# aai-institute/tianshou-fork

Measured on AMD Instinct MI355X. Metric: env-steps/sec through collect+GAE+PPO.learn, higher is better.
Workload: dtype f32 (GAE scan f64)

## Files before the change

include/tsrl.h:

```cpp
#ifndef TSRL_H_
#define TSRL_H_

#include <stdint.h>

#ifdef __cplusplus
extern "C" {
#endif

const char* tsrl_version(void);
const char* tsrl_last_error(void);

int64_t tsrl_gae_workspace_bytes(int64_t n, int64_t row_len);
int64_t tsrl_gae_num_partials(int64_t n, int64_t row_len);
int tsrl_gae(const float* v_s, const float* v_s_next, const double* rew,
             const uint8_t* terminated, const uint8_t* truncated, const uint8_t* end_extra,
             int64_t n, int64_t row_len, const double* value_scale, double gamma,
             double gae_lambda, float* adv_out, float* ret_out, double* adv64_out,
             double* ret64_out, double* ret_partials, void* workspace,
             int64_t workspace_bytes, void* stream);

int tsrl_gae_f64v(const double* v_s, const double* v_s_next, const double* rew,
                  const uint8_t* terminated, const uint8_t* truncated, const uint8_t* end_extra,
                  int64_t n, int64_t row_len, double gamma, double gae_lambda,
                  double* adv64_out, double* ret64_out, void* workspace,
// ... 186 lines not shown
    double eps_clip;
    double dual_clip;
    double vf_coef;
    double ent_coef;
    double adv_eps;
    double b_global;
    int32_t value_clip;
    int32_t norm_adv;
    int32_t objective;
    int32_t pad_;
} tsrl_ppo_params;

int64_t tsrl_ppo_num_partials(int64_t b);
int tsrl_adv_moments(const float* adv, const int64_t* idx, int64_t b, double* partials,
                     void* stream);
int64_t tsrl_adv_moments_seg_parts(int64_t max_seg);
int tsrl_adv_moments_seg(const float* adv, const int64_t* idx, const int64_t* bounds,
                         int64_t nseg, int64_t max_seg, double* partials, double* out,
                         void* stream);
int tsrl_reduce_partials(const double* partials, int64_t nblk, int64_t width, double* out,
                         void* stream);
int tsrl_ppo_gauss_fwd_bwd(const float* mu, const float* log_std, const float* value,
                           const float* act, const float* logp_old, const float* adv,
                           const float* ret, const float* v_s, const int64_t* idx,
                           int64_t b, int64_t act_dim, const double* adv_sums,
                           tsrl_ppo_params p, float* grad_mu, float* grad_value,
                           double* partials, void* stream);
int tsrl_ppo_gauss_finalize(const double* sums, int64_t act_dim, const float* log_std,
                            tsrl_ppo_params p, float* losses, float* grad_log_std,
                            void* stream);
int tsrl_gauss_logp(const float* mu, const float* log_std, const float* act, int64_t b,
                    int64_t act_dim, float* out, void* stream);

int tsrl_ppo_cat_fwd_bwd(const float* x, const float* value, const int64_t* act,
                         const float* logp_old, const float* adv, const float* ret,
                         const float* v_s, const int64_t* idx, int64_t b, int64_t num_actions,
                         int mode, const double* adv_sums, tsrl_ppo_params p, float* grad_x,
                         float* grad_value, double* partials, void* stream);
int tsrl_ppo_cat_finalize(const double* sums, tsrl_ppo_params p, float* losses, void* stream);
int tsrl_cat_logp(const float* x, const int64_t* act, int64_t b, int64_t num_actions, int mode,
                  float* out, void* stream);

int tsrl_cat_gumbel_argmax(const float* logits, const float* u, int64_t n, int64_t num_actions,
                           int64_t* out, void* stream);

typedef struct tsrl_tail_weights {
    const float *w2a, *b2a;
    const float *w2c, *b2c;
    const float *w3a, *b3a;
    const float *w3c, *b3c;
    const float *log_std;
} tsrl_tail_weights;

typedef struct tsrl_tail_grads {
    float *w2a, *b2a, *w2c, *b2c, *w3a, *b3a, *w3c, *b3c;
} tsrl_tail_grads;

int tsrl_mlp_l1_fwd(const float* X, int64_t ldx, const int64_t* idx, int64_t n, int64_t D,
                    const float* Wa, const float* ba, const float* Wc, const float* bc,
                    int act_tanh, float* out, int frag_out, void* stream);
int64_t tsrl_mlp_frag_floats(int64_t n);
int64_t tsrl_mlp_split_bytes(int64_t D);
int tsrl_mlp_split_w(const float* Wa, const float* Wc, int64_t D, void* wsplit, void* stream);
int tsrl_mlp_l1_fwd_x6(const float* X, int64_t ldx, const int64_t* idx, int64_t n, int64_t D,
                       const void* wsplit, const float* ba, const float* bc, int act_tanh,
                       float* out, int frag_out, void* stream);
int64_t tsrl_ppo_tail_workspace_bytes(int64_t n);
int tsrl_ppo_tail_stage(const float* h1frag, int64_t n, const int64_t* idx,
                        const tsrl_tail_weights* w, int64_t act_dim, const float* act,
                        const float* logp_old, const float* adv, const float* ret,
                        const float* v_s, const double* adv_sums, tsrl_ppo_params p, float* dz1,
                        const tsrl_tail_grads* grads, double* sums, void* workspace,
                        int64_t ws_bytes, const float* log_std, float* losses,
                        float* grad_log_std, int stages, void* stream);
int tsrl_ppo_eval(const float* h1frag, int64_t n, const tsrl_tail_weights* w, int64_t act_dim,
                  const float* act, float* value_out, float* logp_out, void* stream);

int64_t tsrl_ppo_eval_fused_workspace_bytes(void);
int tsrl_ppo_eval_fused(const float* X, int64_t ldx, const int64_t* idx, int64_t n, int64_t D,
                        const void* wsplit, const float* ba, const float* bc,
                        const tsrl_tail_weights* wt, int64_t act_dim, const float* act,
                        float* value_out, float* logp_out, void* workspace, int64_t ws_bytes,
                        void* stream);
int64_t tsrl_mlp_dw_workspace_bytes(int64_t n, int64_t D);
int tsrl_mlp_dw(const float* dz1, const float* X, int64_t ldx, const int64_t* idx, int64_t n,
                int64_t D, float* gWa, float* gba, float* gWc, float* gbc, void* workspace,
                int64_t ws_bytes, void* stream);

int64_t tsrl_policy_pack_floats(int64_t D);
int tsrl_policy_pack_l1(const float* W, int64_t D, float* packed, void* stream);
int tsrl_gauss_policy_act(const float* obs, int64_t ldx, int64_t n, int64_t D,
                          const float* w1packed, const float* b1, const float* w2,
                          const float* b2, const float* w3, const float* b3,
                          const float* log_std, int64_t act_dim, const float* eps,
                          int bound_method, const float* low, const float* high, float* act,
                          float* act_remap, void* stream);
int tsrl_gauss_policy_act_rng(const float* obs, int64_t ldx, int64_t n, int64_t D,
                              const float* w1packed, const float* b1, const float* w2,
                              const float* b2, const float* w3, const float* b3,
                              const float* log_std, int64_t act_dim, uint64_t seed,
                              const int64_t* rng_ctr, int64_t* rng_next, int bound_method,
                              const float* low, const float* high, float* act,
                              float* act_remap, void* stream);

int tsrl_nstep_return(const double* rew, const uint8_t* done, const uint8_t* terminated,
                      const int64_t* last_index, const int64_t* lengths, int64_t size,
                      int64_t num, const int64_t* idx, int64_t bsz, int64_t n_step,
                      double gamma, const void* target_q, int64_t X, int f64, void* out,
                      void* stream);
int tsrl_segtree_set(double* tree, int64_t bound, const int64_t* idx, const double* values,
                     int64_t value_stride, int64_t k, int* win, void* stream);
int tsrl_segtree_reduce(const double* tree, int64_t bound, int64_t start, int64_t end,
                        double* out, void* stream);
int tsrl_segtree_prefix_idx(const double* tree, int64_t bound, const void* values, int f64,
                            int64_t k, int64_t* out, void* stream);

typedef struct {
    void* out;
    int64_t off_a, off_c, d, kp;
} tsrl_w1_split;
int64_t tsrl_clip_adam_partials(int64_t n);
int tsrl_clip_adam(float* param, float* grad, float* exp_avg, float* exp_avg_sq, int64_t n,
                   float* step, int64_t nstep, float lr, float beta1, float beta2, float eps,
                   float max_norm, double* partials, float* norm_out, unsigned int* ticket,
                   const float* lr_dev, const tsrl_w1_split* split, int scale_grads,
                   void* stream);
int tsrl_clip_rmsprop(float* param, float* grad, float* square_avg, int64_t n, float* step,
                      int64_t nstep, float lr, float alpha, float eps, float max_norm,
                      double* partials, float* norm_out, unsigned int* ticket,
                      const float* lr_dev, const tsrl_w1_split* split, int scale_grads,
                      void* stream);

int tsrl_dqn_target_q(const float* q_sel, const float* q_eval, int64_t b, int64_t num_actions,
                      int is_double, float* out, void* stream);
int64_t tsrl_dqn_num_partials(int64_t b);
int tsrl_dqn_td_fwd_bwd(const float* q, const int64_t* act, const float* returns,
                        const float* weight, int64_t b, int64_t num_actions, int huber,
                        float* grad_q, float* td_error, double* partials, float* loss,
                        void* stream);
int tsrl_eps_greedy(int64_t* act, const double* u_row, const double* u_act,
                    const uint8_t* mask, double eps, int64_t n, int64_t num_actions,
                    void* stream);

#ifdef __cplusplus
}
#endif
#endif
```

tianshou-fork_amd/csrc/mlp.hip:

```cpp
#include "ppo_loss.h"
#include "x6.h"

namespace tsrl {
namespace {

typedef float f32x16 __attribute__((ext_vector_type(16)));
using x6::bf16x8;
using x6::mfma6;
using x6::NPL;
using x6::split1;
using x6::sw_off;

constexpr int H = 64;
constexpr int HC = 2 * H;
constexpr int NT = HC / 32;
constexpr int AMAX = 32;

__device__ __forceinline__ int rho(int r) { return (r & 3) + 8 * (r >> 2); }

__device__ __forceinline__ f32x16 mfma(float a, float b, f32x16 c) {
    return __builtin_amdgcn_mfma_f32_32x32x2f32(a, b, c, 0, 0, 0);
}

__device__ __forceinline__ f32x16 zero16() {
// ... 749 lines not shown
            __builtin_amdgcn_sched_barrier(0);
            run_net(bt, 0, ua);
            __builtin_amdgcn_sched_barrier(0);
            if (bt + bstep < ntiles) load_unit(bt + bstep, 0, ua);
            __builtin_amdgcn_sched_barrier(0);
            run_net(bt, 1, ub);
            __builtin_amdgcn_sched_barrier(0);
        }
    } else {
        for (; bt < ntiles; bt += bstep) {
            float h1[2][16];
            load_unit(bt, 1, h1);
            run_net(bt, 1, h1);
        }
    }
}

struct TailGrads {
    float *w2a, *b2a, *w2c, *b2c, *w3a, *b3a, *w3c, *b3c;
};

template <typename T>
__device__ __forceinline__ T slab_sum(const T* __restrict__ base, int64_t stride, int nslab,
                                      int64_t i, bool valid, T* sh) {
    const int o = threadIdx.x & 63, g = threadIdx.x >> 6;
    T a0 = 0, a1 = 0, a2 = 0, a3 = 0;
    if (valid) {
        int k = g;
        for (; k + 12 < nslab; k += 16) {
            a0 += base[(int64_t)k * stride + i];
            a1 += base[(int64_t)(k + 4) * stride + i];
            a2 += base[(int64_t)(k + 8) * stride + i];
            a3 += base[(int64_t)(k + 12) * stride + i];
        }
        for (; k < nslab; k += 4) a0 += base[(int64_t)k * stride + i];
    }
    sh[g * 64 + o] = (a0 + a1) + (a2 + a3);
    __syncthreads();
    return ((sh[o] + sh[64 + o]) + sh[128 + o]) + sh[192 + o];
}

struct TailFin {
    const float* log_std;
    float* losses;
    float* grad_log_std;
    float vf_coef, ent_coef;
    double inv_b;
};

__global__ __launch_bounds__(256) void tail_reduce_kernel(const float* __restrict__ slab_f,
                                                          const double* __restrict__ slab_d,
                                                          int nslab, int A, TailGrads g,
                                                          double* __restrict__ sums, TailFin fin) {
    __shared__ float shf[256];
    __shared__ double shd[256];
    const int nfb = (SL_F + 63) / 64;
    if ((int)blockIdx.x < nfb) {
        const int i = blockIdx.x * 64 + (threadIdx.x & 63);
        const float s = slab_sum(slab_f, SL_F, nslab, i, i < SL_F, shf);
        if (threadIdx.x >= 64 || i >= SL_F) return;
        if (i < SL_B2A) g.w2a[i] = s;
        else if (i < SL_W2C) g.b2a[i - SL_B2A] = s;
        else if (i < SL_B2C) g.w2c[i - SL_W2C] = s;
        else if (i < SL_W3A) g.b2c[i - SL_B2C] = s;
        else if (i < SL_B3A) { if (i - SL_W3A < A * H) g.w3a[i - SL_W3A] = s; }
        else if (i < SL_W3C) { if (i - SL_B3A < A) g.b3a[i - SL_B3A] = s; }
        else if (i < SL_B3C) g.w3c[i - SL_W3C] = s;
        else if (i == SL_B3C) g.b3c[0] = s;
    } else {
        const int k0 = threadIdx.x & 63;
        const double s = slab_sum(slab_d, SL_D, nslab, k0, k0 < SL_D, shd);
        if (threadIdx.x < 64 && k0 < 4 + A) sums[k0] = s;
        if (fin.losses) {
            __shared__ double fs[64];
            if (threadIdx.x < 64) fs[k0] = s;
            __syncthreads();
            gauss_finalize(fs, A, fin.log_std, fin.vf_coef, fin.ent_coef, fin.inv_b, fin.losses,
                           fin.grad_log_std);
        }
    }
}

constexpr int DW_COLS = 128;
constexpr int DW_KB = 32;

#ifndef DWX6_OCC
#define DWX6_OCC 2
#endif
__global__ __launch_bounds__(256, DWX6_OCC) void dw_x6_kernel(
    const float* __restrict__ dz, const float* __restrict__ X, int64_t ldx,
    const int64_t* __restrict__ idx, int64_t n, int D, int64_t rows_per_split, int ncolpad,
    int ncolt, float* __restrict__ part) {
    constexpr int PL = 128 * 64;
    __shared__ __attribute__((aligned(16))) char Zi[NPL * PL];
    __shared__ __attribute__((aligned(16))) char Xi[NPL * PL];
    const int t = threadIdx.x;
    const int w = t >> 6, l = t & 63, h = l >> 5, c = l & 31;
    const int G = gridDim.x, b = blockIdx.x;
    const int L = (G & 7) ? b : (b & 7) * (G >> 3) + (b >> 3);
    const int colt = L % ncolt, split = L / ncolt;
    const int col0 = colt * DW_COLS;
    const int64_t r0 = (int64_t)split * rows_per_split;
    const int64_t r1 = min(n, r0 + rows_per_split);
    const int fc = t & 127;
    const int rg = __builtin_amdgcn_readfirstlane(t >> 7);
    const int k = col0 + fc;
    const float ones = k == D ? 1.0f : 0.0f;
    const bool kin = k < D;
    const float* xcol = X + (kin ? k : 0);
    const uint64_t ldx32 = (uint32_t)ldx;
    float zr[16], xr[16];
#define DWX6_LOAD(rb)                                                                       \
    {                                                                                       \
        _Pragma("unroll") for (int q = 0; q < 16; ++q) {                                    \
            const int64_t r = (rb) + 8 * (rg + 2 * (q >> 3)) + (q & 7);                     \
            const int64_t rr = r < r1 ? r : r1 - 1;                                          \
            const int64_t ri = idx ? idx[rr] : rr;                                          \
            zr[q] = dz[rr * HC + fc];                                                       \
            xr[q] = xcol[ri * ldx];                                                         \
        }                                                                                   \
    }
     \
     \
     \
     \
#define DWX6_LOAD_FULL(rb)                                                                  \
    {                                                                                       \
        _Pragma("unroll") for (int g_ = 0; g_ < 2; ++g_) {                                  \
            const int64_t rg0_ = (rb) + 8 * (rg + 2 * g_);                                  \
            const float* zb_ = dz + rg0_ * HC + fc;                                         \
            const int64_t* ib_ = idx + rg0_;                                                \
            _Pragma("unroll") for (int j_ = 0; j_ < 8; ++j_) {                              \
                zr[8 * g_ + j_] = zb_[j_ * HC];                                             \
                const uint64_t ri_ = (uint32_t)ib_[j_];                                     \
                xr[8 * g_ + j_] = xcol[ri_ * ldx32];                                        \
            }                                                                               \
        }                                                                                   \
    }
     \
     \
#define DWX6_STORE(rb, FULL)                                                                \
    {                                                                                       \
        _Pragma("unroll") for (int g = 0; g < 2; ++g) {                                     \
            bf16x8 zp[NPL], xp[NPL];                                                        \
            _Pragma("unroll") for (int j = 0; j < 8; ++j) {                                 \
                const bool lv = (FULL) || (rb) + 8 * (rg + 2 * g) + j < r1;                 \
                const float zv = lv ? zr[8 * g + j] : 0.0f;                                 \
                const float xv = lv ? (kin ? xr[8 * g + j] : ones) : 0.0f;                  \
                __bf16 a0, a1, a2;                                                          \
                split1(zv, a0, a1, a2);                                                     \
                zp[0][j] = a0;                                                              \
                zp[1][j] = a1;                                                              \
                zp[2][j] = a2;                                                              \
                split1(xv, a0, a1, a2);                                                     \
                xp[0][j] = a0;                                                              \
                xp[1][j] = a1;                                                              \
                xp[2][j] = a2;                                                              \
            }                                                                               \
            const int off = sw_off(fc, rg + 2 * g);                                         \
            _Pragma("unroll") for (int p = 0; p < NPL; ++p) {                               \
                *reinterpret_cast<bf16x8*>(Zi + p * PL + off) = zp[p];                      \
                *reinterpret_cast<bf16x8*>(Xi + p * PL + off) = xp[p];                      \
            }                                                                               \
        }                                                                                   \
    }
    f32x16 acc[NT];
#pragma unroll
    for (int i = 0; i < NT; ++i) acc[i] = zero16();
    const int64_t nchunk = r1 > r0 ? (r1 - r0 + DW_KB - 1) / DW_KB : 0;
    if (nchunk > 0) {
        DWX6_LOAD(r0)
        DWX6_STORE(r0, false)
    }
    __syncthreads();
    for (int64_t ch = 0; ch < nchunk; ++ch) {
        if (ch + 1 < nchunk) {
            const int64_t rb = r0 + (ch + 1) * DW_KB;
            if (idx && rb + DW_KB <= r1)
                DWX6_LOAD_FULL(rb)
            else
                DWX6_LOAD(rb)
        }
#pragma unroll
        for (int s = 0; s < 2; ++s) {
            bf16x8 b[NPL];
            const int xo = sw_off(32 * w + c, 2 * s + h);
#pragma unroll
            for (int p = 0; p < NPL; ++p) b[p] = *reinterpret_cast<const bf16x8*>(Xi + p * PL + xo);
#pragma unroll
            for (int i = 0; i < NT; ++i) {
                bf16x8 a[NPL];
                const int zo = sw_off(32 * i + c, 2 * s + h);
#pragma unroll
                for (int p = 0; p < NPL; ++p)
                    a[p] = *reinterpret_cast<const bf16x8*>(Zi + p * PL + zo);
                acc[i] = mfma6(a, b, acc[i]);
            }
        }
        if (ch + 1 < nchunk) {
            __syncthreads();
            const int64_t rb = r0 + (ch + 1) * DW_KB;
            if (rb + DW_KB <= r1)
                DWX6_STORE(rb, true)
            else
                DWX6_STORE(rb, false)
            __syncthreads();
        }
    }
#undef DWX6_LOAD
#undef DWX6_LOAD_FULL
#undef DWX6_STORE
    float* o = part + (int64_t)split * HC * ncolpad;
#pragma unroll
    for (int i = 0; i < NT; ++i)
#pragma unroll
        for (int r = 0; r < 16; ++r)
            o[(int64_t)(32 * i + rho(r) + 4 * h) * ncolpad + col0 + 32 * w + c] = acc[i][r];
}

__global__ __launch_bounds__(256) void dw_reduce_kernel(const float* __restrict__ part,
                                                        int nsplit, int ncolpad, int D,
                                                        float* __restrict__ gWa,
                                                        float* __restrict__ gba,
                                                        float* __restrict__ gWc,
                                                        float* __restrict__ gbc) {
    __shared__ float sh[256];
    const int64_t i = (int64_t)blockIdx.x * 64 + (threadIdx.x & 63);
    const int64_t total = (int64_t)HC * ncolpad;
    const int f = (int)(i / ncolpad), k = (int)(i - (int64_t)f * ncolpad);
    const bool valid = i < total && k <= D;
    const float s = slab_sum(part, total, nsplit, i, valid, sh);
    if (threadIdx.x >= 64 || !valid) return;
    if (k == D) {
        if (f < H) gba[f] = s; else gbc[f - H] = s;
    } else {
        if (f < H) gWa[(int64_t)f * D + k] = s; else gWc[(int64_t)(f - H) * D + k] = s;
    }
}

int tail_grid(int64_t n) {
    const int64_t tiles = (n + 15) / 16;
    const int64_t g = (tiles + T16_NW - 1) / T16_NW;
    return (int)std::min<int64_t>(g, 256);
}

int dw_nsplit(int64_t n) {
    int64_t s = std::max<int64_t>(1, std::min<int64_t>(170, n / 64));
    if (s >= 8) s &= ~int64_t(7);
    return (int)s;
}

}
}

using namespace tsrl;

extern "C" int tsrl_mlp_l1_fwd(const float* X, int64_t ldx, const int64_t* idx, int64_t n,
                               int64_t D, const float* Wa, const float* ba, const float* Wc,
                               const float* bc, int act_tanh, float* out, int frag_out,
                               void* stream) {
    TSRL_CHECK_ARG(n >= 0 && D > 0 && ldx >= D, "tsrl_mlp_l1_fwd: bad sizes");
    if (n == 0) return 0;
    TSRL_CHECK_ARG(X && Wa && ba && Wc && bc && out, "tsrl_mlp_l1_fwd: null pointer");
    TSRL_CHECK_ARG(aligned16(X) && ldx % 4 == 0 && aligned16(Wa) && aligned16(Wc) && D % 4 == 0 &&
                       aligned16(out),
                   "tsrl_mlp_l1_fwd: X/W/out must be 16-byte aligned with D, ldx multiples of 4");
    const unsigned grid = (unsigned)((n + L1_ROWS - 1) / L1_ROWS);
    hipLaunchKernelGGL(l1_fwd_kernel, dim3(grid), dim3(256), 0, as_stream(stream), X, ldx, idx, n,
                       (int)D, Wa, ba, Wc, bc, act_tanh, out, frag_out);
    TSRL_LAUNCH_CHECK("tsrl_mlp_l1_fwd");
    return 0;
}

extern "C" int64_t tsrl_mlp_frag_floats(int64_t n) {
    return ((n + L1_ROWS - 1) / L1_ROWS) * L1_ROWS * HC;
}

extern "C" int64_t tsrl_ppo_tail_workspace_bytes(int64_t n) {
    const int g = tail_grid(n);
    return (int64_t)g * (SL_F * (int64_t)sizeof(float) + SL_D * (int64_t)sizeof(double)) + 256;
}

extern "C" int tsrl_ppo_tail_stage(const float* h1frag, int64_t n, const int64_t* idx,
                                   const tsrl_tail_weights* wt, int64_t act_dim, const float* act,
                                   const float* logp_old, const float* adv, const float* ret,
                                   const float* v_s, const double* adv_sums, tsrl_ppo_params prm,
                                   float* dz1, const tsrl_tail_grads* grads, double* sums,
                                   void* workspace, int64_t ws_bytes, const float* log_std,
                                   float* losses, float* grad_log_std, int stages, void* stream) {
    TSRL_CHECK_ARG((log_std && losses && grad_log_std) || (!log_std && !losses && !grad_log_std),
                   "tsrl_ppo_tail_stage: log_std/losses/grad_log_std all set or all null");
    TSRL_CHECK_ARG((stages >= 1 && stages <= 3) || stages == 4 || stages == 8,
                   "tsrl_ppo_tail_stage: stages must be 1, 2, 3, 4 or 8");
    TSRL_CHECK_ARG(n > 0 && act_dim > 0 && act_dim <= AMAX,
                   "tsrl_ppo_tail_stage: need n > 0 and 0 < act_dim <= %d", AMAX);
    TSRL_CHECK_ARG(h1frag && wt && grads && act && adv && ret && dz1 && sums && workspace,
                   "tsrl_ppo_tail_stage: null pointer");
    TSRL_CHECK_ARG(objective_args_ok(prm, logp_old),
                   "tsrl_ppo_tail_stage: objective 0 needs logp_old; objective 1 takes no "
                   "norm_adv, value_clip or dual_clip");
    TSRL_CHECK_ARG(!prm.value_clip || v_s, "tsrl_ppo_tail_stage: value_clip needs v_s");
    TSRL_CHECK_ARG(!prm.norm_adv || adv_sums, "tsrl_ppo_tail_stage: norm_adv needs adv_sums");
    TSRL_CHECK_ARG(prm.b_global >= 1.0, "tsrl_ppo_tail_stage: b_global < 1");
    TSRL_CHECK_ARG(ws_bytes >= tsrl_ppo_tail_workspace_bytes(n),
                   "tsrl_ppo_tail_stage: workspace too small");
    TSRL_CHECK_ARG(aligned16(h1frag) && aligned16(dz1),
                   "tsrl_ppo_tail_stage: h1frag/dz1 not 16-byte aligned");
    const int g = tail_grid(n);
    float* slab_f = reinterpret_cast<float*>(workspace);
    uintptr_t dptr = reinterpret_cast<uintptr_t>(slab_f + (int64_t)g * SL_F);
    dptr = (dptr + 15) & ~(uintptr_t)15;
    double* slab_d = reinterpret_cast<double*>(dptr);
    TailWeights w{wt->w2a, wt->b2a, wt->w2c, wt->b2c, wt->w3a, wt->b3a, wt->w3c, wt->b3c,
                  wt->log_std};
    const LossParams lp = make_loss_params(prm);
    const int A = (int)act_dim;
    if (stages & (1 | 4)) {
        auto actor = prm.objective == OBJ_A2C ? ppo_tail16_kernel<0, OBJ_A2C>
                                              : ppo_tail16_kernel<0, OBJ_PPO>;
        hipLaunchKernelGGL(actor, dim3(g), dim3(T16_TPB), 0, as_stream(stream), h1frag, n, idx,
                           w, act, logp_old, adv, ret, v_s, adv_sums, lp, A, dz1, slab_f, slab_d);
        TSRL_LAUNCH_CHECK("tsrl_ppo_tail_stage(actor)");
    }
    if (stages & (1 | 8)) {
        hipLaunchKernelGGL((ppo_tail16_kernel<1, OBJ_PPO>), dim3(g), dim3(T16_TPB), 0,
                           as_stream(stream), h1frag, n, idx, w, act, logp_old, adv, ret, v_s,
                           adv_sums, lp, A, dz1, slab_f, slab_d);
        TSRL_LAUNCH_CHECK("tsrl_ppo_tail_stage(critic)");
    }
    if (!(stages & 2)) return 0;
    TailGrads gg{grads->w2a, grads->b2a, grads->w2c, grads->b2c, grads->w3a, grads->b3a,
                 grads->w3c, grads->b3c};
    const TailFin fin{log_std, losses, grad_log_std, lp.vf_coef, lp.ent_coef, lp.inv_b};
    hipLaunchKernelGGL(tail_reduce_kernel, dim3((SL_F + 63) / 64 + 1), dim3(256), 0,
                       as_stream(stream), slab_f, slab_d, g, A, gg, sums, fin);
    TSRL_LAUNCH_CHECK("tsrl_ppo_tail_stage(reduce)");
    return 0;
}

extern "C" int64_t tsrl_mlp_dw_workspace_bytes(int64_t n, int64_t D) {
    const int ncolpad = (int)(((D + 1 + DW_COLS - 1) / DW_COLS) * DW_COLS);
    const int nsplit = dw_nsplit(n);
    return (int64_t)nsplit * HC * ncolpad * (int64_t)sizeof(float);
}

extern "C" int tsrl_mlp_dw(const float* dz1, const float* X, int64_t ldx, const int64_t* idx,
                           int64_t n, int64_t D, float* gWa, float* gba, float* gWc, float* gbc,
                           void* workspace, int64_t ws_bytes, void* stream) {
    TSRL_CHECK_ARG(n > 0 && D > 0 && ldx >= D, "tsrl_mlp_dw: bad sizes");
    TSRL_CHECK_ARG(dz1 && X && gWa && gba && gWc && gbc && workspace, "tsrl_mlp_dw: null pointer");
    TSRL_CHECK_ARG(aligned16(dz1) && aligned16(X) && ldx % 4 == 0 && ldx >= (D + 3) / 4 * 4 && ldx < (int64_t(1) << 32),
                   "tsrl_mlp_dw: dz1/X must be 16-byte aligned, ldx a multiple of 4 and >= "
                   "roundup(D, 4) (columns D.. of the padding read as data-free)");
    TSRL_CHECK_ARG(ws_bytes >= tsrl_mlp_dw_workspace_bytes(n, D), "tsrl_mlp_dw: workspace too small");
    const int ncolt = (int)((D + 1 + DW_COLS - 1) / DW_COLS);
    const int ncolpad = ncolt * DW_COLS;
    const int nsplit = dw_nsplit(n);
    const int64_t rps = ((n + nsplit - 1) / nsplit + DW_KB - 1) / DW_KB * DW_KB;
    float* part = reinterpret_cast<float*>(workspace);
    hipLaunchKernelGGL(dw_x6_kernel, dim3(ncolt * nsplit), dim3(256), 0, as_stream(stream),
                       dz1, X, ldx, idx, n, (int)D, rps, ncolpad, ncolt, part);
    TSRL_LAUNCH_CHECK("tsrl_mlp_dw");
    const int64_t outs = (int64_t)HC * ncolpad;
    hipLaunchKernelGGL(dw_reduce_kernel, dim3((unsigned)((outs + 63) / 64)), dim3(256), 0,
                       as_stream(stream), part, nsplit, ncolpad, (int)D, gWa, gba, gWc, gbc);
    TSRL_LAUNCH_CHECK("tsrl_mlp_dw(reduce)");
    return 0;
}

extern "C" int tsrl_ppo_eval(const float* h1frag, int64_t n, const tsrl_tail_weights* wt,
                             int64_t act_dim, const float* act, float* value_out,
                             float* logp_out, void* stream) {
    TSRL_CHECK_ARG(n >= 0 && act_dim > 0 && act_dim <= AMAX, "tsrl_ppo_eval: bad sizes");
    if (n == 0) return 0;
    TSRL_CHECK_ARG(h1frag && wt && value_out && (!logp_out || act),
                   "tsrl_ppo_eval: null pointer");
    TSRL_CHECK_ARG(aligned16(h1frag), "tsrl_ppo_eval: h1frag not 16-byte aligned");
    TailWeights w{wt->w2a, wt->b2a, wt->w2c, wt->b2c, wt->w3a, wt->b3a, wt->w3c, wt->b3c,
                  wt->log_std};
    const int64_t tiles = (n + 31) / 32;
    const unsigned g = (unsigned)std::min<int64_t>((tiles + 3) / 4, 1024);
    if (logp_out)
        hipLaunchKernelGGL(eval_tail_kernel<true>, dim3(g), dim3(256), 0, as_stream(stream), h1frag,
                           n, w, (int)act_dim, act, value_out, logp_out);
    else
        hipLaunchKernelGGL(eval_tail_kernel<false>, dim3(g), dim3(256), 0, as_stream(stream),
                           h1frag, n, w, (int)act_dim, act, value_out, logp_out);
    TSRL_LAUNCH_CHECK("tsrl_ppo_eval");
    return 0;
}
```

tianshou-fork_amd/tianshou_amd/_C.py:

```python
import ctypes
import os

import torch

_HERE = os.path.dirname(os.path.abspath(__file__))
LIB_PATH = os.environ.get("TSRL_LIB_PATH") or os.path.join(_HERE, "lib", "libtsrl.so")

_i64 = ctypes.c_int64
_u64 = ctypes.c_uint64
_p = ctypes.c_void_p
_d = ctypes.c_double
_f = ctypes.c_float
_i32 = ctypes.c_int32


class AddArgs(ctypes.Structure):
    _fields_ = [
        ("ids", _p), ("ptr", _p), ("next_rel", _p), ("offset", _p), ("k", _i64),
        ("uniform_rel", _i64), ("uniform_next", _i64), ("rel_dev", _p), ("ring_size", _i64),
        ("obs_src", _p), ("obs_dst", _p), ("obs_row_bytes", _i64),
        ("obs_next_src", _p), ("obs_next_dst", _p), ("cur_obs", _p), ("obs_dim", _i64),
        ("norm_mean", _p), ("norm_var", _p), ("norm_eps", _f), ("norm_clip", _f),
        ("obs_next_src_raw", _p), ("obs_next_dst_raw", _p),
        ("act_src", _p), ("act_dst", _p), ("act_row_bytes", _i64),
# ... 85 lines not shown
    "tsrl_rms_sum_partials2": ([_p, _p, _p, _i64, _i64, _i64, _p, _p], ctypes.c_int),
    "tsrl_rms_norm_rows": ([_p, _p, _i64, _i64, _p, _p, _f, _f, _p, _p], ctypes.c_int),
    "tsrl_buffer_add": ([ctypes.POINTER(AddArgs), _p], ctypes.c_int),
    "tsrl_collect_pack_floats": ([_i64], _i64),
    "tsrl_collect_pack_w1": ([_p, _i64, _p, _p], ctypes.c_int),
    "tsrl_collect_workspace_bytes": ([_i64, _i64], _i64),
    "tsrl_collect_box_step": ([ctypes.POINTER(CollectArgs), _p], ctypes.c_int),
    "tsrl_collect_rms_finalize": ([ctypes.POINTER(CollectArgs), _p], ctypes.c_int),
    "tsrl_collect_totals_offset": ([_i64], _i64),
    "tsrl_collect_spec_step": ([ctypes.POINTER(CollectArgs), _i32, _p], ctypes.c_int),
    "tsrl_collect_xpipe_finalize": ([ctypes.POINTER(CollectArgs), _p], ctypes.c_int),
    "tsrl_rms_exact_stats_bytes": ([_i64], _i64),
    "tsrl_rms_exact_stats": ([_p, _i64, _p, _p, _i64, _p, _p], ctypes.c_int),
    "tsrl_rms_exact_stats_n": ([_i32, _p, _p, _p, _i64, _i64, _p, _p], ctypes.c_int),
    "tsrl_rms_exact_stats_max_steps": ([], ctypes.c_int),
    "tsrl_gather_rows": ([_p, _i64, _p, _i64, _p, _p], ctypes.c_int),
    "tsrl_gather_rows_pitched": ([_p, _i64, _i64, _p, _i64, _p, _p], ctypes.c_int),
    "tsrl_np_shuffle_draws": ([_p, _p, _i64, _p], ctypes.c_int),
    "tsrl_shuffle_apply_workspace_bytes": ([_i64], _i64),
    "tsrl_shuffle_apply": ([_p, _i64, _p, _p, _i64, _p], ctypes.c_int),
    "tsrl_ring_step_index": ([_p, _i64, _p, _p, _p, _i64, _i64, ctypes.c_int, _p, _p],
                             ctypes.c_int),
    "tsrl_stack_gather_pitched": ([_p, _i64, _i64, _p, _i64, _i64, _p, _p, _p, _i64, _i64, _p,
                                   _p, _p], ctypes.c_int),
    "tsrl_stack_gather": ([_p, _i64, _p, _i64, _i64, _p, _p, _p, _i64, _i64, _p, _p, _p],
                          ctypes.c_int),
    "tsrl_frames_to_f32_nhwc": ([_p, _i64, _i64, _i64, _p, _p, _p], ctypes.c_int),
    "tsrl_dqn_conv1_fwd": ([_p, _i64, _p, _p, _i64, _i64, _i64, _i64, _p, _f, ctypes.c_int, _p,
                            _p],
                           ctypes.c_int),
    "tsrl_dqn_conv2_dgrad": ([_p, _i64, _p, _i64, _i64, _i64, _i64, _p, _p, _p], ctypes.c_int),
    "tsrl_relu_bwd_rows_workspace_bytes": ([_i64, _i64], _i64),
    "tsrl_relu_bwd_rows": ([_p, _p, _p, _i64, _i64, _p, _p, _i64, _p], ctypes.c_int),
    "tsrl_bias_relu_rows": ([_p, _p, _i64, _i64, _p], ctypes.c_int),
    "tsrl_dqn_conv1_wgrad_workspace_bytes": ([_i64], _i64),
    "tsrl_dqn_conv1_wgrad": ([_p, _i64, _p, _p, _f, _p, _p, _p, _i64, _p], ctypes.c_int),
    "tsrl_nstep_return": ([_p, _p, _p, _p, _p, _i64, _i64, _p, _i64, _i64, _d, _p, _i64,
                           ctypes.c_int, _p, _p], ctypes.c_int),
    "tsrl_clip_adam_partials": ([_i64], _i64),
    "tsrl_clip_adam": ([_p, _p, _p, _p, _i64, _p, _i64, _f, _f, _f, _f, _f, _p, _p, _p, _p,
                        ctypes.POINTER(W1Split), ctypes.c_int, _p],
                       ctypes.c_int),
    "tsrl_clip_rmsprop": ([_p, _p, _p, _i64, _p, _i64, _f, _f, _f, _f, _p, _p, _p, _p,
                           ctypes.POINTER(W1Split), ctypes.c_int, _p], ctypes.c_int),
    "tsrl_segtree_set": ([_p, _i64, _p, _p, _i64, _i64, _p, _p], ctypes.c_int),
    "tsrl_segtree_reduce": ([_p, _i64, _i64, _i64, _p, _p], ctypes.c_int),
    "tsrl_segtree_prefix_idx": ([_p, _i64, _p, ctypes.c_int, _i64, _p, _p], ctypes.c_int),
    "tsrl_sum_rows_workspace_bytes": ([_i64, _i64], _i64),
    "tsrl_sum_rows_f32": ([_p, _i64, _i64, _p, _p, _i64, _p], ctypes.c_int),
    "tsrl_ppo_num_partials": ([_i64], _i64),
    "tsrl_adv_moments": ([_p, _p, _i64, _p, _p], ctypes.c_int),
    "tsrl_reduce_partials": ([_p, _i64, _i64, _p, _p], ctypes.c_int),
    "tsrl_adv_moments_seg_parts": ([_i64], _i64),
    "tsrl_adv_moments_seg": ([_p, _p, _p, _i64, _i64, _p, _p, _p], ctypes.c_int),
    "tsrl_ppo_gauss_fwd_bwd": ([_p, _p, _p, _p, _p, _p, _p, _p, _p, _i64, _i64, _p, PPOParams,
                                _p, _p, _p, _p], ctypes.c_int),
    "tsrl_ppo_gauss_finalize": ([_p, _i64, _p, PPOParams, _p, _p, _p], ctypes.c_int),
    "tsrl_gauss_logp": ([_p, _p, _p, _i64, _i64, _p, _p], ctypes.c_int),
    "tsrl_ppo_cat_fwd_bwd": ([_p, _p, _p, _p, _p, _p, _p, _p, _i64, _i64, ctypes.c_int, _p,
                              PPOParams, _p, _p, _p, _p], ctypes.c_int),
    "tsrl_ppo_cat_finalize": ([_p, PPOParams, _p, _p], ctypes.c_int),
    "tsrl_cat_logp": ([_p, _p, _i64, _i64, ctypes.c_int, _p, _p], ctypes.c_int),
    "tsrl_cat_gumbel_argmax": ([_p, _p, _i64, _i64, _p, _p], ctypes.c_int),
    "tsrl_rms_exact_update": ([_p, _p, _i64, _p, _p, _i64, _i64, _p, _p, _p, _p, _p, _p, _p],
                              ctypes.c_int),
    "tsrl_np_shuffle_draws_mt": ([_p, _p, _i64, _p, ctypes.c_int], ctypes.c_int),
    "tsrl_mlp_l1_fwd": ([_p, _i64, _p, _i64, _i64, _p, _p, _p, _p, ctypes.c_int, _p,
                         ctypes.c_int, _p], ctypes.c_int),
    "tsrl_mlp_frag_floats": ([_i64], _i64),
    "tsrl_mlp_split_bytes": ([_i64], _i64),
    "tsrl_mlp_split_w": ([_p, _p, _i64, _p, _p], ctypes.c_int),
    "tsrl_mlp_l1_fwd_x6": ([_p, _i64, _p, _i64, _i64, _p, _p, _p, ctypes.c_int, _p,
                            ctypes.c_int, _p], ctypes.c_int),
    "tsrl_ppo_tail_workspace_bytes": ([_i64], _i64),
    "tsrl_ppo_tail_stage": ([_p, _i64, _p, ctypes.POINTER(TailWeights), _i64, _p, _p, _p, _p,
                             _p, _p, PPOParams, _p, ctypes.POINTER(TailGrads), _p, _p, _i64, _p,
                             _p, _p, ctypes.c_int, _p], ctypes.c_int),
    "tsrl_ppo_eval": ([_p, _i64, ctypes.POINTER(TailWeights), _i64, _p, _p, _p, _p],
                      ctypes.c_int),
    "tsrl_ppo_eval_fused_workspace_bytes": ([], _i64),
    "tsrl_ppo_eval_fused": ([_p, _i64, _p, _i64, _i64, _p, _p, _p, ctypes.POINTER(TailWeights),
                             _i64, _p, _p, _p, _p, _i64, _p], ctypes.c_int),
    "tsrl_mlp_dw_workspace_bytes": ([_i64, _i64], _i64),
    "tsrl_policy_pack_floats": ([_i64], _i64),
    "tsrl_gauss_policy_act_rng": ([_p, _i64, _i64, _i64, _p, _p, _p, _p, _p, _p, _p, _i64, _u64,
                                   _p, _p, ctypes.c_int, _p, _p, _p, _p, _p], ctypes.c_int),
    "tsrl_policy_pack_l1": ([_p, _i64, _p, _p], ctypes.c_int),
    "tsrl_gauss_policy_act": ([_p, _i64, _i64, _i64, _p, _p, _p, _p, _p, _p, _p, _i64, _p,
                               ctypes.c_int, _p, _p, _p, _p, _p], ctypes.c_int),
    "tsrl_mlp_dw": ([_p, _p, _i64, _p, _i64, _i64, _p, _p, _p, _p, _p, _i64, _p], ctypes.c_int),
    "tsrl_dqn_target_q": ([_p, _p, _i64, _i64, ctypes.c_int, _p, _p], ctypes.c_int),
    "tsrl_dqn_num_partials": ([_i64], _i64),
    "tsrl_dqn_td_fwd_bwd": ([_p, _p, _p, _p, _i64, _i64, ctypes.c_int, _p, _p, _p, _p, _p],
                            ctypes.c_int),
    "tsrl_eps_greedy": ([_p, _p, _p, _p, _d, _i64, _i64, _p], ctypes.c_int),
}

EXPORTED = tuple(_SIGS)
_LIB = None


class TsrlError(RuntimeError):
    pass


def lib():
    global _LIB
    if _LIB is None:
        if not os.path.exists(LIB_PATH):
            raise ImportError(
                f"libtsrl.so not found at {LIB_PATH}: build it with "
                "`python -c 'import __graft_entry__ as g; g.build()'` (hipcc, gfx950)")
        L = ctypes.CDLL(LIB_PATH)
        for name, (args, res) in _SIGS.items():
            fn = getattr(L, name)
            fn.argtypes = args
            fn.restype = res
        _LIB = L
    return _LIB


def check(rc, what=""):
    if rc != 0:
        msg = lib().tsrl_last_error().decode(errors="replace")
        raise TsrlError(f"{what or 'libtsrl'} failed (hipError {rc}): {msg}")


def stream_ptr(device=None):
    return torch.cuda.current_stream(device).cuda_stream


def ptr(t, dtype=None):
    if t is None:
        return None
    if not isinstance(t, torch.Tensor):
        raise TypeError(f"expected a torch.Tensor, got {type(t)}")
    if t.device.type != "cuda":
        raise TsrlError(f"libtsrl kernels need HIP device tensors; got a tensor on {t.device}")
    if dtype is not None and t.dtype != dtype:
        raise TypeError(f"expected dtype {dtype}, got {t.dtype}")
    if not t.is_contiguous():
        raise ValueError("libtsrl kernels need contiguous tensors")
    return t.data_ptr()


def ptr_rows(t):
    if t is None:
        return None
    if t.dim() >= 2 and t[0].is_contiguous() and t.stride(0) >= t[0].numel():
        if t.device.type != "cuda":
            raise TsrlError(f"libtsrl kernels need HIP device tensors; got a tensor on {t.device}")
        return t.data_ptr()
    return ptr(t)
```

Baseline: 68.20 million.

## Widen MLP weight-gradient kernel to multi-column-tile blocks with double-buffered LDS

Replaces the dW kernel with a templated wide kernel in which one block covers up to three 128-column tiles. The dz tile is loaded and split once per block and reused across those column tiles instead of being reloaded per tile. The chunk size drops to 16 rows, with double-buffered LDS images, register prefetch two chunks ahead, and split/MFMA interleaving via sched_group_barrier, so only one barrier is needed per chunk. The cost is larger blocks (up to 768 threads), more LDS and registers per block, a possible second launch for leftover tiles, and a new plan API.

```diff
diff --git a/include/tsrl.h b/include/tsrl.h
--- a/include/tsrl.h
+++ b/include/tsrl.h
@@ -292,6 +292,8 @@
                         const tsrl_tail_weights* wt, int64_t act_dim, const float* act,
                         float* value_out, float* logp_out, void* workspace, int64_t ws_bytes,
                         void* stream);
+int tsrl_mlp_dw_plan(int64_t n, int64_t D, int64_t* nsplit, int64_t* rows_per_split,
+                     int64_t* col_tiles, int64_t* chunk_rows);
 int64_t tsrl_mlp_dw_workspace_bytes(int64_t n, int64_t D);
 int tsrl_mlp_dw(const float* dz1, const float* X, int64_t ldx, const int64_t* idx, int64_t n,
                 int64_t D, float* gWa, float* gba, float* gWc, float* gbc, void* workspace,
diff --git a/tianshou-fork_amd/csrc/mlp.hip b/tianshou-fork_amd/csrc/mlp.hip
--- a/tianshou-fork_amd/csrc/mlp.hip
+++ b/tianshou-fork_amd/csrc/mlp.hip
@@ -855,134 +855,189 @@
 }
 
 constexpr int DW_COLS = 128;
-constexpr int DW_KB = 32;
-
-#ifndef DWX6_OCC
-#define DWX6_OCC 2
-#endif
-__global__ __launch_bounds__(256, DWX6_OCC) void dw_x6_kernel(
+constexpr int DW_KB = 16;
+constexpr int DW_MAXCT = 3;
+
+__device__ __forceinline__ int dw_off(int row, int q) {
+    return row * 32 + 16 * (q ^ ((row >> 2) & 1) ^ ((row >> 3) & 1));
+}
+
+template <int CT>
+__global__ __launch_bounds__(256 * CT) void dw_wide_kernel(
     const float* __restrict__ dz, const float* __restrict__ X, int64_t ldx,
     const int64_t* __restrict__ idx, int64_t n, int D, int64_t rows_per_split, int ncolpad,
-    int ncolt, float* __restrict__ part) {
-    constexpr int PL = 128 * 64;
-    __shared__ __attribute__((aligned(16))) char Zi[NPL * PL];
-    __shared__ __attribute__((aligned(16))) char Xi[NPL * PL];
+    int colt0, int ngrp, float* __restrict__ part) {
+    constexpr int NC = DW_COLS * CT;
+    constexpr int NS = 2;
+    constexpr int ZPL = HC * 2 * DW_KB;
+    constexpr int XPL = NC * 2 * DW_KB;
+    constexpr int BUF = NPL * (ZPL + XPL);
+    __shared__ __attribute__((aligned(16))) char img[2 * BUF];
     const int t = threadIdx.x;
     const int w = t >> 6, l = t & 63, h = l >> 5, c = l & 31;
-    const int G = gridDim.x, b = blockIdx.x;
-    const int L = (G & 7) ? b : (b & 7) * (G >> 3) + (b >> 3);
-    const int colt = L % ncolt, split = L / ncolt;
-    const int col0 = colt * DW_COLS;
+    const int grp = blockIdx.x % ngrp, split = blockIdx.x / ngrp;
+    const int col0 = (colt0 + grp * CT) * DW_COLS;
     const int64_t r0 = (int64_t)split * rows_per_split;
     const int64_t r1 = min(n, r0 + rows_per_split);
-    const int fc = t & 127;
-    const int rg = __builtin_amdgcn_readfirstlane(t >> 7);
-    const int k = col0 + fc;
+    const int xc = t % NC;
+    const int xrg = __builtin_amdgcn_readfirstlane(t / NC);
+    const bool zt = __builtin_amdgcn_readfirstlane(w) < 4;
+    const int zf = t & 127;
+    const int zrg = __builtin_amdgcn_readfirstlane((t >> 7) & 1);
+    const int k = col0 + xc;
     const float ones = k == D ? 1.0f : 0.0f;
     const bool kin = k < D;
-    const float* xcol = X + (kin ? k : 0);
+    const uint32_t kxb = (kin ? k : 0) * 4u, zfb = zf * 4u;
+    auto at = [](const float* row, uint32_t byte_off) __attribute__((always_inline)) {
+        return *reinterpret_cast<const float*>(reinterpret_cast<const char*>(row) + byte_off);
+    };
     const uint64_t ldx32 = (uint32_t)ldx;
-    float zr[16], xr[16];
-#define DWX6_LOAD(rb)                                                                       \
-    {                                                                                       \
-        _Pragma("unroll") for (int q = 0; q < 16; ++q) {                                    \
-            const int64_t r = (rb) + 8 * (rg + 2 * (q >> 3)) + (q & 7);                     \
-            const int64_t rr = r < r1 ? r : r1 - 1;                                          \
-            const int64_t ri = idx ? idx[rr] : rr;                                          \
-            zr[q] = dz[rr * HC + fc];                                                       \
-            xr[q] = xcol[ri * ldx];                                                         \
-        }                                                                                   \
-    }
-     \
-     \
-     \
-     \
-#define DWX6_LOAD_FULL(rb)                                                                  \
-    {                                                                                       \
-        _Pragma("unroll") for (int g_ = 0; g_ < 2; ++g_) {                                  \
-            const int64_t rg0_ = (rb) + 8 * (rg + 2 * g_);                                  \
-            const float* zb_ = dz + rg0_ * HC + fc;                                         \
-            const int64_t* ib_ = idx + rg0_;                                                \
-            _Pragma("unroll") for (int j_ = 0; j_ < 8; ++j_) {                              \
-                zr[8 * g_ + j_] = zb_[j_ * HC];                                             \
-                const uint64_t ri_ = (uint32_t)ib_[j_];                                     \
-                xr[8 * g_ + j_] = xcol[ri_ * ldx32];                                        \
-            }                                                                               \
-        }                                                                                   \
-    }
-     \
-     \
-#define DWX6_STORE(rb, FULL)                                                                \
-    {                                                                                       \
-        _Pragma("unroll") for (int g = 0; g < 2; ++g) {                                     \
-            bf16x8 zp[NPL], xp[NPL];                                                        \
-            _Pragma("unroll") for (int j = 0; j < 8; ++j) {                                 \
-                const bool lv = (FULL) || (rb) + 8 * (rg + 2 * g) + j < r1;                 \
-                const float zv = lv ? zr[8 * g + j] : 0.0f;                                 \
-                const float xv = lv ? (kin ? xr[8 * g + j] : ones) : 0.0f;                  \
-                __bf16 a0, a1, a2;                                                          \
-                split1(zv, a0, a1, a2);                                                     \
-                zp[0][j] = a0;                                                              \
-                zp[1][j] = a1;                                                              \
-                zp[2][j] = a2;                                                              \
-                split1(xv, a0, a1, a2);                                                     \
-                xp[0][j] = a0;                                                              \
-                xp[1][j] = a1;                                                              \
-                xp[2][j] = a2;                                                              \
-            }                                                                               \
-            const int off = sw_off(fc, rg + 2 * g);                                         \
-            _Pragma("unroll") for (int p = 0; p < NPL; ++p) {                               \
-                *reinterpret_cast<bf16x8*>(Zi + p * PL + off) = zp[p];                      \
-                *reinterpret_cast<bf16x8*>(Xi + p * PL + off) = xp[p];                      \
-            }                                                                               \
-        }                                                                                   \
-    }
+    int wsz[2], wsx[2], rdz[2], rdx[2];
+#pragma unroll
+    for (int q = 0; q < 2; ++q) {
+        wsz[q] = q * BUF + dw_off(zf, zrg);
+        wsx[q] = q * BUF + NPL * ZPL + dw_off(xc, xrg);
+        rdz[q] = q * BUF + dw_off(c, h);
+        rdx[q] = q * BUF + NPL * ZPL + dw_off(32 * w + c, h);
+        asm volatile("" : "+v"(wsz[q]), "+v"(wsx[q]), "+v"(rdz[q]), "+v"(rdx[q]));
+    }
+
+    auto load_full = [&](float (&xs)[8], float (&zs)[8], int64_t rb, bool zt) __attribute__((always_inline)) {
+        const int64_t* ib = idx + rb + 8 * xrg;
+#pragma unroll
+        for (int j = 0; j < 8; ++j) {
+            const uint64_t ri = (uint32_t)ib[j];
+            xs[j] = at(X + ri * ldx32, kxb);
+        }
+        if (zt) {
+            const float* zb = dz + (rb + 8 * zrg) * HC;
+#pragma unroll
+            for (int j = 0; j < 8; ++j) zs[j] = at(zb + j * HC, zfb);
+        }
+    };
+    auto load = [&](float (&xs)[8], float (&zs)[8], int64_t rb, bool zt) __attribute__((always_inline)) {
+        if (idx && rb + DW_KB <= r1) {
+            load_full(xs, zs, rb, zt);
+            return;
+        }
+        if (idx) {
+#pragma unroll
+            for (int j = 0; j < 8; ++j) {
+                const int64_t r = rb + 8 * xrg + j;
+                xs[j] = at(X + idx[r < r1 ? r : r1 - 1] * ldx, kxb);
+            }
+        } else {
+#pragma unroll
+            for (int j = 0; j < 8; ++j) {
+                const int64_t r = rb + 8 * xrg + j;
+                xs[j] = at(X + (r < r1 ? r : r1 - 1) * ldx, kxb);
+            }
+        }
+        if (zt) {
+#pragma unroll
+            for (int j = 0; j < 8; ++j) {
+                const int64_t r = rb + 8 * zrg + j;
+                zs[j] = at(dz + (r < r1 ? r : r1 - 1) * HC, zfb);
+            }
+        }
+    };
+    auto stage_z = [&](const float (&zs)[8], int64_t rb, int buf, bool full) __attribute__((always_inline)) {
+        bf16x8 zp[NPL];
+#pragma unroll
+        for (int j = 0; j < 8; ++j) {
+            const float zv = (full || rb + 8 * zrg + j < r1) ? zs[j] : 0.0f;
+            __bf16 a0, a1, a2;
+            split1(zv, a0, a1, a2);
+            zp[0][j] = a0;
+            zp[1][j] = a1;
+            zp[2][j] = a2;
+        }
+#pragma unroll
+        for (int p = 0; p < NPL; ++p)
+            *reinterpret_cast<bf16x8*>(img + wsz[buf] + p * ZPL) = zp[p];
+    };
+    auto split_x = [&](const float (&xs)[8], int j, bf16x8 (&xp)[NPL], bool ex) __attribute__((always_inline)) {
+        const float xv = ex ? (kin ? xs[j] : ones) : 0.0f;
+        __bf16 a0, a1, a2;
+        split1(xv, a0, a1, a2);
+        xp[0][j] = a0;
+        xp[1][j] = a1;
+        xp[2][j] = a2;
+    };
+    auto store_x = [&](const bf16x8 (&xp)[NPL], int buf) __attribute__((always_inline)) {
+#pragma unroll
+        for (int p = 0; p < NPL; ++p)
+            *reinterpret_cast<bf16x8*>(img + wsx[buf] + p * XPL) = xp[p];
+    };
+
     f32x16 acc[NT];
 #pragma unroll
     for (int i = 0; i < NT; ++i) acc[i] = zero16();
+    auto mma = [&](int rz, int rx, const float (&xs)[8], int wx, bool ex) __attribute__((always_inline)) {
+        bf16x8 b[NPL], xp[NPL];
+#pragma unroll
+        for (int p = 0; p < NPL; ++p)
+            b[p] = *reinterpret_cast<const bf16x8*>(img + rx + p * XPL);
+#pragma unroll
+        for (int i = 0; i < NT; ++i) {
+            bf16x8 a[NPL];
+#pragma unroll
+            for (int p = 0; p < NPL; ++p)
+                a[p] = *reinterpret_cast<const bf16x8*>(img + rz + p * ZPL + i * 32 * 32);
+            acc[i] = mfma6(a, b, acc[i]);
+            split_x(xs, 2 * i, xp, ex);
+            split_x(xs, 2 * i + 1, xp, ex);
+#pragma unroll
+            for (int m = 0; m < 6; ++m) {
+                __builtin_amdgcn_sched_group_barrier(0x008, 1, 0);
+                __builtin_amdgcn_sched_group_barrier(0x002, 4, 0);
+            }
+            __builtin_amdgcn_sched_barrier(0);
+        }
+#pragma unroll
+        for (int p = 0; p < NPL; ++p)
+            *reinterpret_cast<bf16x8*>(img + wx + p * XPL) = xp[p];
+    };
+
     const int64_t nchunk = r1 > r0 ? (r1 - r0 + DW_KB - 1) / DW_KB : 0;
-    if (nchunk > 0) {
-        DWX6_LOAD(r0)
-        DWX6_STORE(r0, false)
+    float xs[NS][8], zs[NS][8];
+#pragma unroll
+    for (int q = 0; q < NS; ++q)
+        if (r0 + q * DW_KB < r1) load(xs[q], zs[q], r0 + q * DW_KB, zt);
+    {
+        if (zt) stage_z(zs[0], r0, 0, false);
+        bf16x8 xp[NPL];
+#pragma unroll
+        for (int j = 0; j < 8; ++j) split_x(xs[0], j, xp, r0 < r1);
+        store_x(xp, 0);
+        if (r0 + NS * DW_KB < r1) load(xs[0], zs[0], r0 + NS * DW_KB, zt);
     }
     __syncthreads();
-    for (int64_t ch = 0; ch < nchunk; ++ch) {
-        if (ch + 1 < nchunk) {
-            const int64_t rb = r0 + (ch + 1) * DW_KB;
-            if (idx && rb + DW_KB <= r1)
-                DWX6_LOAD_FULL(rb)
+    auto iter = [&](int64_t q, int cur, float (&x)[8], float (&z)[8], bool fast) __attribute__((always_inline)) {
+        const int64_t rb = r0 + (q + 1) * DW_KB;
+        if (zt) {
+            if (fast || rb + DW_KB <= r1)
+                stage_z(z, rb, cur ^ 1, true);
             else
-                DWX6_LOAD(rb)
-        }
-#pragma unroll
-        for (int s = 0; s < 2; ++s) {
-            bf16x8 b[NPL];
-            const int xo = sw_off(32 * w + c, 2 * s + h);
-#pragma unroll
-            for (int p = 0; p < NPL; ++p) b[p] = *reinterpret_cast<const bf16x8*>(Xi + p * PL + xo);
-#pragma unroll
-            for (int i = 0; i < NT; ++i) {
-                bf16x8 a[NPL];
-                const int zo = sw_off(32 * i + c, 2 * s + h);
-#pragma unroll
-                for (int p = 0; p < NPL; ++p)
-                    a[p] = *reinterpret_cast<const bf16x8*>(Zi + p * PL + zo);
-                acc[i] = mfma6(a, b, acc[i]);
-            }
-        }
-        if (ch + 1 < nchunk) {
-            __syncthreads();
-            const int64_t rb = r0 + (ch + 1) * DW_KB;
-            if (rb + DW_KB <= r1)
-                DWX6_STORE(rb, true)
-            else
-                DWX6_STORE(rb, false)
-            __syncthreads();
-        }
-    }
-#undef DWX6_LOAD
-#undef DWX6_LOAD_FULL
-#undef DWX6_STORE
+                stage_z(z, rb, cur ^ 1, false);
+        }
+        mma(rdz[cur], rdx[cur], x, wsx[cur ^ 1], fast || rb < r1);
+        if (fast)
+            load_full(x, z, rb + NS * DW_KB, zt);
+        else if (rb + NS * DW_KB < r1)
+            load(x, z, rb + NS * DW_KB, zt);
+        __syncthreads();
+    };
+    int64_t ch = 0;
+    if (idx)
+        for (; r0 + (ch + 2 * NS + 1) * DW_KB <= r1; ch += NS) {
+#pragma unroll
+            for (int u = 0; u < NS; ++u) iter(ch + u, u & 1, xs[(u + 1) % NS], zs[(u + 1) % NS], true);
+        }
+    for (; ch < nchunk; ch += NS) {
+#pragma unroll
+        for (int u = 0; u < NS; ++u) iter(ch + u, u & 1, xs[(u + 1) % NS], zs[(u + 1) % NS], false);
+    }
     float* o = part + (int64_t)split * HC * ncolpad;
 #pragma unroll
     for (int i = 0; i < NT; ++i)
@@ -1017,10 +1072,37 @@
     return (int)std::min<int64_t>(g, 256);
 }
 
-int dw_nsplit(int64_t n) {
-    int64_t s = std::max<int64_t>(1, std::min<int64_t>(170, n / 64));
-    if (s >= 8) s &= ~int64_t(7);
-    return (int)s;
+struct DwPlan {
+    int ncolt, ngrp, ct, nbig, nsplit;
+    int64_t rps;
+};
+
+DwPlan dw_plan(int64_t n, int64_t D) {
+    DwPlan p;
+    p.ncolt = (int)((D + 1 + DW_COLS - 1) / DW_COLS);
+    p.ngrp = (p.ncolt + DW_MAXCT - 1) / DW_MAXCT;
+    p.ct = (p.ncolt + p.ngrp - 1) / p.ngrp;
+    p.nbig = p.ncolt % p.ngrp ? p.ncolt % p.ngrp : p.ngrp;
+    int64_t ns = std::max<int64_t>(1, std::min<int64_t>(170, n / 64));
+    if (ns >= 8) ns &= ~int64_t(7);
+    p.nsplit = (int)ns;
+    p.rps = ((n + p.nsplit - 1) / p.nsplit + 31) / 32 * 32;
+    return p;
+}
+
+template <int CT>
+void dw_launch(const DwPlan& p, int colt0, int ngrp, const float* dz1, const float* X,
+               int64_t ldx, const int64_t* idx, int64_t n, int D, float* part, void* stream) {
+    hipLaunchKernelGGL(dw_wide_kernel<CT>, dim3((unsigned)(p.nsplit * ngrp)), dim3(256 * CT), 0,
+                       as_stream(stream), dz1, X, ldx, idx, n, D, p.rps, p.ncolt * DW_COLS, colt0,
+                       ngrp, part);
+}
+
+void dw_launch_ct(int ct, const DwPlan& p, int colt0, int ngrp, const float* dz1, const float* X,
+                  int64_t ldx, const int64_t* idx, int64_t n, int D, float* part, void* stream) {
+    if (ct == 1) dw_launch<1>(p, colt0, ngrp, dz1, X, ldx, idx, n, D, part, stream);
+    else if (ct == 2) dw_launch<2>(p, colt0, ngrp, dz1, X, ldx, idx, n, D, part, stream);
+    else dw_launch<3>(p, colt0, ngrp, dz1, X, ldx, idx, n, D, part, stream);
 }
 
 }
@@ -1111,10 +1193,20 @@
     return 0;
 }
 
+extern "C" int tsrl_mlp_dw_plan(int64_t n, int64_t D, int64_t* nsplit, int64_t* rows_per_split,
+                                int64_t* col_tiles, int64_t* chunk_rows) {
+    TSRL_CHECK_ARG(n > 0 && D > 0, "tsrl_mlp_dw_plan: bad sizes");
+    const DwPlan p = dw_plan(n, D);
+    if (nsplit) *nsplit = p.nsplit;
+    if (rows_per_split) *rows_per_split = p.rps;
+    if (col_tiles) *col_tiles = p.ct;
+    if (chunk_rows) *chunk_rows = DW_KB;
+    return 0;
+}
+
 extern "C" int64_t tsrl_mlp_dw_workspace_bytes(int64_t n, int64_t D) {
-    const int ncolpad = (int)(((D + 1 + DW_COLS - 1) / DW_COLS) * DW_COLS);
-    const int nsplit = dw_nsplit(n);
-    return (int64_t)nsplit * HC * ncolpad * (int64_t)sizeof(float);
+    const DwPlan p = dw_plan(n, D);
+    return (int64_t)p.nsplit * HC * p.ncolt * DW_COLS * (int64_t)sizeof(float);
 }
 
 extern "C" int tsrl_mlp_dw(const float* dz1, const float* X, int64_t ldx, const int64_t* idx,
@@ -1126,17 +1218,19 @@
                    "tsrl_mlp_dw: dz1/X must be 16-byte aligned, ldx a multiple of 4 and >= "
                    "roundup(D, 4) (columns D.. of the padding read as data-free)");
     TSRL_CHECK_ARG(ws_bytes >= tsrl_mlp_dw_workspace_bytes(n, D), "tsrl_mlp_dw: workspace too small");
-    const int ncolt = (int)((D + 1 + DW_COLS - 1) / DW_COLS);
-    const int ncolpad = ncolt * DW_COLS;
-    const int nsplit = dw_nsplit(n);
-    const int64_t rps = ((n + nsplit - 1) / nsplit + DW_KB - 1) / DW_KB * DW_KB;
+    const DwPlan p = dw_plan(n, D);
+    const int ncolpad = p.ncolt * DW_COLS;
     float* part = reinterpret_cast<float*>(workspace);
-    hipLaunchKernelGGL(dw_x6_kernel, dim3(ncolt * nsplit), dim3(256), 0, as_stream(stream),
-                       dz1, X, ldx, idx, n, (int)D, rps, ncolpad, ncolt, part);
+    dw_launch_ct(p.ct, p, 0, p.nbig, dz1, X, ldx, idx, n, (int)D, part, stream);
     TSRL_LAUNCH_CHECK("tsrl_mlp_dw");
+    if (p.nbig < p.ngrp) {
+        dw_launch_ct(p.ct - 1, p, p.nbig * p.ct, p.ngrp - p.nbig, dz1, X, ldx, idx, n, (int)D,
+                     part, stream);
+        TSRL_LAUNCH_CHECK("tsrl_mlp_dw");
+    }
     const int64_t outs = (int64_t)HC * ncolpad;
     hipLaunchKernelGGL(dw_reduce_kernel, dim3((unsigned)((outs + 63) / 64)), dim3(256), 0,
-                       as_stream(stream), part, nsplit, ncolpad, (int)D, gWa, gba, gWc, gbc);
+                       as_stream(stream), part, p.nsplit, ncolpad, (int)D, gWa, gba, gWc, gbc);
     TSRL_LAUNCH_CHECK("tsrl_mlp_dw(reduce)");
     return 0;
 }
diff --git a/tianshou-fork_amd/tianshou_amd/_C.py b/tianshou-fork_amd/tianshou_amd/_C.py
--- a/tianshou-fork_amd/tianshou_amd/_C.py
+++ b/tianshou-fork_amd/tianshou_amd/_C.py
@@ -191,6 +191,7 @@
     "tsrl_ppo_eval_fused": ([_p, _i64, _p, _i64, _i64, _p, _p, _p, ctypes.POINTER(TailWeights),
                              _i64, _p, _p, _p, _p, _i64, _p], ctypes.c_int),
     "tsrl_mlp_dw_workspace_bytes": ([_i64, _i64], _i64),
+    "tsrl_mlp_dw_plan": ([_i64, _i64, _p, _p, _p, _p], ctypes.c_int),
     "tsrl_policy_pack_floats": ([_i64], _i64),
     "tsrl_gauss_policy_act_rng": ([_p, _i64, _i64, _i64, _p, _p, _p, _p, _p, _p, _p, _i64, _u64,
                                    _p, _p, ctypes.c_int, _p, _p, _p, _p, _p], ctypes.c_int),
```

New measurement: 67.70 million. About the same (-0.7%).
